# dalek-cryptography/curve25519-dalek

Hardware: NVIDIA H100
Metric: Pippenger MSM points/sec (higher is better)
Workload: dtype exact integers: f64 limbs (radix 2^51, FP64 pipe) in the bucket kernel, u32 limbs (radix 2^25.5) elsewhere

## Files before the change

### curve25519_dalek_b200/csrc/fe64.cuh

```cuda
#pragma once
#include <stdint.h>

#include "fe.cuh"

struct fe64 { double v[5]; };

#define FE64_E52 0x4330000000000000LL
#define FE64_TWO52 4503599627370496.0
#define FE64_TWO51 2251799813685248.0

#if defined(__CUDA_ARCH__)
#define FE64_DEV 1
#else
#define FE64_DEV 0
#include <assert.h>
#include <math.h>
#include <string.h>
#endif

FE_HD void fe64_0(fe64 &h) { for (int i = 0; i < 5; i++) h.v[i] = 0.0; }
FE_HD void fe64_1(fe64 &h) { h.v[0] = 1.0; for (int i = 1; i < 5; i++) h.v[i] = 0.0; }

FE_HD void fe64_add(fe64 &h, const fe64 &f, const fe64 &g)
{
// ... 207 lines not shown
    }
}

FE_HD void fe64_to_fe(fe &o, const fe64 &f)
{
    uint64_t l[5];
#pragma unroll
    for (int k = 0; k < 5; k++) {
        long long r = (long long)f.v[k];
        l[k] = (uint64_t)(r + (k == 0 ? (1LL << 54) - 152 : (1LL << 54) - 8));
    }
    uint64_t c[10];
#pragma unroll
    for (int i = 0; i < 5; i++) { c[2 * i] = l[i] & FE_M26; c[2 * i + 1] = l[i] >> 26; }
    fe_carry64(o, c);
}

FE_HD void fe64_from_fe(fe64 &h, const fe &f)
{
    uint32_t w[8];
    fe_tobytes_words(w, f);
    fe64 t; fe64_frombytes_words(t, w);
    fe64_carry(h, t);
}

FE_HD void fe64_pow22501(fe64 &t19, fe64 &t3, const fe64 &z)
{
    fe64 t0, t1, t2, t5, t6, t7, t9, t13, t15;
    fe64_sq(t0, z);
    fe64_sqn(t1, t0, 2);
// ... 33 lines not shown
```

### curve25519_dalek_b200/csrc/msm.cu

```cuda
#include <algorithm>
#include <cstdio>
#include <utility>
#include <vector>

#include "../../include/dalek_b200.h"
#include "engine.h"
#include "ge64.cuh"
#include "warp4.cuh"
#include "warp4_f64.cuh"

static inline unsigned cdiv(size_t a, unsigned b) { return (unsigned)((a + b - 1) / b); }

int ws_reserve(dalek_b200_ctx *ctx, DevBuf &b, size_t bytes)
{
    if (bytes <= b.cap) return 0;
    if (b.p) { cudaFree(b.p); b.p = nullptr; b.cap = 0; }
    size_t want = bytes + bytes / 8 + 256;
    cudaError_t e = cudaMalloc(&b.p, want);
    if (e != cudaSuccess) {
        ctx->last_error = std::string("cudaMalloc: ") + cudaGetErrorString(e);
        (void)cudaGetLastError();
        return DALEK_E_NOMEM;
    }
    b.cap = want;
// ... 46 lines not shown
    ge_niels nl; ge_affine_to_niels(nl, P.X, P.Y);
    ge_niels_packed pk; ge_niels_pack(pk, nl);
    out[i] = pk;
}

#define PREP_THREADS 256
#define PREP_PER_THREAD 4
#define PREP_GROUP (PREP_THREADS * PREP_PER_THREAD)
#define PREP_NW (PREP_THREADS / 32)

__device__ __forceinline__ void load_coord_f64(fe64 &h, const uint64_t *__restrict__ src)
{
    uint64_t l[5];
#pragma unroll
    for (int k = 0; k < 5; k++) l[k] = __ldg(src + k);
    fe t; fe_from_limbs51(t, l);
    fe64_from_fe_limbs(h, t);
}
__device__ __forceinline__ void store_coord(uint4 *o, const fe64 &v, uint32_t ok, uint32_t c)
{
    fe f;
    uint32_t w[8];
    fe64_to_fe(f, v); fe_tobytes_words(w, f);
#pragma unroll
    for (int q = 0; q < 8; q++) w[q] = ok ? w[q] : (q == 0 ? c : 0u);
    o[0] = make_uint4(w[0], w[1], w[2], w[3]);
    o[1] = make_uint4(w[4], w[5], w[6], w[7]);
}
__device__ __forceinline__ uint32_t load_z(fe64 &h, const uint64_t *__restrict__ in, size_t i)
{
    uint64_t l[5];
#pragma unroll
    for (int k = 0; k < 5; k++) l[k] = __ldg(in + 20 * i + 10 + k);
    fe t; fe_from_limbs51(t, l);
    fe64_from_fe_limbs(h, t);
    return 1u - (uint32_t)fe_iszero(t);
}
__device__ __forceinline__ void fe64_shfl_up(fe64 &o, const fe64 &f, int d)
{
#pragma unroll
    for (int k = 0; k < 5; k++) o.v[k] = __shfl_up_sync(0xffffffffu, f.v[k], d);
}
__device__ __forceinline__ void fe64_shfl_down(fe64 &o, const fe64 &f, int d)
{
#pragma unroll
    for (int k = 0; k < 5; k++) o.v[k] = __shfl_down_sync(0xffffffffu, f.v[k], d);
}
__device__ __forceinline__ void fe64_shfl_xor(fe64 &o, const fe64 &f, int m)
{
#pragma unroll
    for (int k = 0; k < 5; k++) o.v[k] = __shfl_xor_sync(0xffffffffu, f.v[k], m);
// ... 43 lines not shown
        if (INVERT) {
            const w20_role r = w20_roles();
            const double inv = w20_invert(w20_limb(all, r.i), r);
#pragma unroll
            for (uint32_t k = 0; k < 5; k++) t.v[k] = w20_shfl(inv, k);
        } else {
            t = *tot_inv;
        }
        fe64_mul(t, t, b); fe64_mul(t, t, a);
        if (lane < nw) s_warp[lane] = t;
    }
    __syncthreads();
    fe64_mul(inv, s_warp[warp], below); fe64_mul(inv, inv, above);
}

__global__ void __launch_bounds__(PREP_THREADS, 2)
k_prep_zprod(const uint64_t *__restrict__ in, fe64 *__restrict__ prod, size_t n)
{
    __shared__ fe64 s_warp[PREP_NW];
    const uint32_t tid = threadIdx.x, lane = tid & 31, warp = tid >> 5;
    const size_t g0 = (size_t)blockIdx.x * PREP_GROUP + tid;
    fe64 z[PREP_PER_THREAD], acc, t;
    uint32_t ok[PREP_PER_THREAD];
#pragma unroll
    for (int k = 0; k < PREP_PER_THREAD; k++) {
        const size_t i = g0 + (size_t)k * PREP_THREADS;
        if (i < n) ok[k] = load_z(z[k], in, i); else { ok[k] = 0; fe64_1(z[k]); }
    }
    acc = z[0];
    if (!ok[0]) fe64_1(acc);
#pragma unroll
    for (int k = 1; k < PREP_PER_THREAD; k++) { fe64_mul(t, acc, z[k]); fe64_cmov(acc, t, ok[k]); }
    warp_product(t, acc, 32);
    if (lane == 0) s_warp[warp] = t;
    __syncthreads();
    if (warp == 0) {
        if (lane < PREP_NW) acc = s_warp[lane]; else fe64_1(acc);
        warp_product(t, acc, PREP_NW);
        if (lane == 0) prod[blockIdx.x] = t;
    }
}

__global__ void __launch_bounds__(PREP_THREADS)
k_prep_invert(fe64 *__restrict__ prod, fe64 *__restrict__ pre, uint32_t G)
{
    __shared__ fe64 s_warp[PREP_NW];
    const uint32_t per = (G + blockDim.x - 1) / blockDim.x, b = min(threadIdx.x * per, G), e = min(b + per, G);
    fe64 acc, inv, t;
    fe64_1(acc);
    for (uint32_t k = b; k < e; k++) { fe64_mul(acc, acc, prod[k]); pre[k] = acc; }
    block_inverse<true>(inv, acc, s_warp, nullptr);
    for (uint32_t k = e; k-- > b;) {
        const fe64 x = prod[k];
        if (k > b) fe64_mul(t, inv, pre[k - 1]); else t = inv;
        prod[k] = t;
        fe64_mul(inv, inv, x);
    }
}

__global__ void __launch_bounds__(PREP_THREADS, 2)
k_prep_finish(const uint64_t *__restrict__ in, const fe64 *__restrict__ ginv, ge_niels_packed *__restrict__ out, size_t n)
{
    __shared__ fe64 s_warp[PREP_NW];
    __shared__ fe64 s_pre[PREP_PER_THREAD - 1][PREP_THREADS];
    const uint32_t tid = threadIdx.x;
    const size_t g0 = (size_t)blockIdx.x * PREP_GROUP + tid;
    fe64 acc, inv;
    uint32_t nz = 0;
    fe64_1(acc);
#pragma unroll 1
    for (int k = 0; k < PREP_PER_THREAD; k++) {
        const size_t i = g0 + (size_t)k * PREP_THREADS;
// ... 53 lines not shown
int msm_prepare_points_on(dalek_b200_ctx *ctx, cudaStream_t st, const void *d_in, int point_fmt, size_t n, void *d_out, int *d_bad,
                          int kind)
{
    if (n == 0) return 0;
    if (point_fmt == DALEK_POINTS_COMPRESSED) {
        if (ctx->opt_decompress_f64) k_prep_compressed<1><<<cdiv(n, 128), 128, 0, st>>>((const uint4 *)d_in, (ge_niels_packed *)d_out, n, d_bad);
        else k_prep_compressed<0><<<cdiv(n, 128), 128, 0, st>>>((const uint4 *)d_in, (ge_niels_packed *)d_out, n, d_bad);
    } else if (point_fmt == DALEK_POINTS_RISTRETTO) {
        if (ctx->opt_decompress_f64) k_prep_ristretto<1><<<cdiv(n, 128), 128, 0, st>>>((const uint32_t *)d_in, (ge_niels_packed *)d_out, n, d_bad);
        else k_prep_ristretto<0><<<cdiv(n, 128), 128, 0, st>>>((const uint32_t *)d_in, (ge_niels_packed *)d_out, n, d_bad);
    } else if (kind == PK_PNIELS) {
        k_prep_extended_pniels<<<cdiv(n, 128), 128, 0, st>>>((const uint64_t *)d_in, (ge_pniels_packed *)d_out, n);
    } else {
        const unsigned G = cdiv(n, PREP_GROUP);
        int rc;
        if ((rc = ws_reserve(ctx, ctx->ws[WS_PREP_PROD], 2 * (size_t)G * sizeof(fe64)))) return rc;
        fe64 *prod = (fe64 *)ctx->ws[WS_PREP_PROD].p;
        k_prep_zprod<<<G, PREP_THREADS, 0, st>>>((const uint64_t *)d_in, prod, n);
        k_prep_invert<<<1, PREP_THREADS, 0, st>>>(prod, prod + G, G);
        k_prep_finish<<<G, PREP_THREADS, 0, st>>>((const uint64_t *)d_in, prod, (ge_niels_packed *)d_out, n);
        ctx->launches += 2;
    }
    ctx->launches++;
    CUDA_TRY(ctx, cudaGetLastError());
    return 0;
}

int msm_prepare_points(dalek_b200_ctx *ctx, const void *d_in, int point_fmt, size_t n, void *d_out, int *d_bad, int kind)
{
    return msm_prepare_points_on(ctx, ctx->stream, d_in, point_fmt, n, d_out, d_bad, kind);
}

int msm_window_count_for_bits(int c) { return 256 / c + 1; }

int msm_choose_window_bits(const dalek_b200_ctx *ctx, size_t n)
{
// ... 270 lines not shown
            warp_claim(out, r[u].y, k < m);
        }
    }
    __syncthreads();
    for (uint32_t f = threadIdx.x; f < nf; f += SORT_THREADS)
        if (out[f]) out[f] = h[f] + atomicAdd(&fill[b0 + f], out[f]);
    __syncthreads();
    for (uint32_t k0 = 0; k0 < m; k0 += SORT_THREADS) {
        const uint32_t k = k0 + threadIdx.x;
        const uint2 r = k < m ? recs[k] : make_uint2(0, 0);
        const uint32_t pos = warp_claim(out, r.y, k < m);
        if (k < m) dst[pos] = r.x;
    }
}

#define SCAN_PART 4096u
__global__ void __launch_bounds__(1024) k_scan_partial(const uint32_t *__restrict__ in, uint32_t nbuckets, uint32_t parts,
                                                       uint32_t *__restrict__ part_sums)
{
    __shared__ uint32_t sh[32];
    uint32_t w = blockIdx.x / parts, part = blockIdx.x % parts;
    const uint32_t *src = in + (size_t)w * nbuckets;
    uint32_t base = part * SCAN_PART + threadIdx.x * 4, sum = 0;
#pragma unroll
    for (int k = 0; k < 4; k++) if (base + k < nbuckets) sum += src[base + k];
    for (int d = 16; d > 0; d >>= 1) sum += __shfl_down_sync(0xffffffffu, sum, d);
    if ((threadIdx.x & 31) == 0) sh[threadIdx.x >> 5] = sum;
    __syncthreads();
    if (threadIdx.x < 32) {
        uint32_t v = sh[threadIdx.x];
        for (int d = 16; d > 0; d >>= 1) v += __shfl_down_sync(0xffffffffu, v, d);
        if (threadIdx.x == 0) part_sums[blockIdx.x] = v;
    }
}
__global__ void k_scan_bases(uint32_t *__restrict__ part_sums, uint32_t parts)
{
    if (threadIdx.x) return;
    uint32_t *p = part_sums + (size_t)blockIdx.x * parts, run = 0;
    for (uint32_t k = 0; k < parts; k++) { uint32_t v = p[k]; p[k] = run; run += v; }
}
__global__ void __launch_bounds__(1024) k_scan_apply(const uint32_t *__restrict__ in, const uint32_t *__restrict__ part_base,
                                                     uint32_t nbuckets, uint32_t parts, uint32_t *__restrict__ out)
{
    __shared__ uint32_t sh[32];
    uint32_t w = blockIdx.x / parts, part = blockIdx.x % parts;
    const uint32_t *src = in + (size_t)w * nbuckets;
    uint32_t *dst = out + (size_t)w * nbuckets;
    uint32_t base = part * SCAN_PART + threadIdx.x * 4;
    uint32_t v[4], sum = 0;
#pragma unroll
    for (int k = 0; k < 4; k++) { v[k] = base + k < nbuckets ? src[base + k] : 0; sum += v[k]; }
    uint32_t incl = sum;
    for (int d = 1; d < 32; d <<= 1) { uint32_t t = __shfl_up_sync(0xffffffffu, incl, d); if ((threadIdx.x & 31) >= d) incl += t; }
    if ((threadIdx.x & 31) == 31) sh[threadIdx.x >> 5] = incl;
    __syncthreads();
    if (threadIdx.x < 32) {
        uint32_t x = sh[threadIdx.x], inc2 = x;
        for (int d = 1; d < 32; d <<= 1) { uint32_t t = __shfl_up_sync(0xffffffffu, inc2, d); if (threadIdx.x >= d) inc2 += t; }
        sh[threadIdx.x] = inc2 - x;
    }
    __syncthreads();
    uint32_t run = part_base[blockIdx.x] + sh[threadIdx.x >> 5] + incl - sum;
#pragma unroll
    for (int k = 0; k < 4; k++) { if (base + k < nbuckets) dst[base + k] = run; run += v[k]; }
}

#define TASK_LEN_MIN 64u
static uint32_t msm_task_len(size_t n, int nwin, uint32_t nb)
{
    const size_t total_buckets = (size_t)nwin * nb;
    const size_t want = total_buckets >= ((size_t)1 << 18) ? 2 * (n / nb) : (n * (size_t)nwin) >> 18;
    uint32_t len = TASK_LEN_MIN;
    while (len < want && len < (1u << 22)) len <<= 1;
    return len;
}
#ifndef ACC_MIN_BLOCKS
#define ACC_MIN_BLOCKS 4
#endif

__global__ void k_task_count(const uint32_t *__restrict__ counts, uint32_t total_buckets, uint32_t task_len,
                             uint32_t *__restrict__ ntasks, uint32_t *__restrict__ heavy)
{
    uint32_t t = blockIdx.x * blockDim.x + threadIdx.x;
    if (t >= total_buckets) return;
    uint32_t c = counts[t];
    uint32_t k = c <= task_len ? 1u : (c + task_len - 1) / task_len;
    ntasks[t] = k;
    if (k > 1) heavy[1 + atomicAdd(&heavy[0], 1u)] = t;
}

__global__ void k_task_bases(const uint32_t *__restrict__ ntasks, const uint32_t *__restrict__ task_off, uint32_t nbuckets,
                             int nwin, uint32_t *__restrict__ win_base )
{
    if (blockIdx.x || threadIdx.x) return;
    uint32_t run = 0;
    for (int w = 0; w < nwin; w++) {
        win_base[w] = run;
        size_t last = (size_t)w * nbuckets + nbuckets - 1;
        run += task_off[last] + ntasks[last];
    }
    win_base[nwin] = run;
}

__global__ void k_task_fill(const uint32_t *__restrict__ ntasks, const uint32_t *__restrict__ task_off,
                            const uint32_t *__restrict__ win_base, uint32_t nbuckets, uint32_t total_buckets,
                            uint2 *__restrict__ tasks)
{
    uint32_t t = blockIdx.x * blockDim.x + threadIdx.x;
    if (t >= total_buckets) return;
    uint32_t w = t / nbuckets;
    uint32_t base = win_base[w] + task_off[t], k = ntasks[t];
    for (uint32_t j = 0; j < k; j++) tasks[base + j] = make_uint2(t, j);
}

#define TASK_BINS 256u
__device__ __forceinline__ uint32_t task_key(uint32_t len, uint32_t task_len)
{
    return (uint32_t)(((uint64_t)len * (TASK_BINS - 1) + task_len - 1) / task_len);
}
__device__ __forceinline__ uint32_t task_length(const uint2 tk, const uint32_t *__restrict__ counts, uint32_t task_len)
{
    return min(task_len, counts[tk.x] - tk.y * task_len);
}

__global__ void __launch_bounds__(256)
k_task_hist(const uint2 *__restrict__ tasks, const uint32_t *__restrict__ counts, const uint32_t *__restrict__ total_ptr,
            uint32_t task_len, uint32_t *__restrict__ hist)
{
    __shared__ uint32_t sh[TASK_BINS];
    sh[threadIdx.x] = 0;
    __syncthreads();
    const uint32_t p = blockIdx.x * blockDim.x + threadIdx.x;
    if (p < *total_ptr) atomicAdd(&sh[task_key(task_length(tasks[p], counts, task_len), task_len)], 1u);
    __syncthreads();
    if (sh[threadIdx.x]) atomicAdd(&hist[threadIdx.x], sh[threadIdx.x]);
}

__global__ void __launch_bounds__(256) k_task_scan(const uint32_t *__restrict__ hist, uint32_t *__restrict__ start)
{
    __shared__ uint32_t sh[TASK_BINS];
    const uint32_t k = TASK_BINS - 1 - threadIdx.x;
    sh[threadIdx.x] = hist[k];
    __syncthreads();
    for (uint32_t d = 1; d < TASK_BINS; d <<= 1) {
        uint32_t v = threadIdx.x >= d ? sh[threadIdx.x - d] : 0;
        __syncthreads();
        sh[threadIdx.x] += v;
        __syncthreads();
    }
    start[k] = sh[threadIdx.x] - hist[k];
}

__global__ void __launch_bounds__(256)
k_task_scatter(const uint2 *__restrict__ tasks, const uint32_t *__restrict__ counts, const uint32_t *__restrict__ total_ptr,
               uint32_t task_len, const uint32_t *__restrict__ start, uint32_t *__restrict__ cursor, uint32_t *__restrict__ order)
{
    __shared__ uint32_t cnt[TASK_BINS], base[TASK_BINS];
    cnt[threadIdx.x] = 0;
    __syncthreads();
    const uint32_t p = blockIdx.x * blockDim.x + threadIdx.x;
    const bool live = p < *total_ptr;
    uint32_t key = 0, rank = 0;
    if (live) { key = task_key(task_length(tasks[p], counts, task_len), task_len); rank = atomicAdd(&cnt[key], 1u); }
    __syncthreads();
    if (cnt[threadIdx.x]) base[threadIdx.x] = start[threadIdx.x] + atomicAdd(&cursor[threadIdx.x], cnt[threadIdx.x]);
    __syncthreads();
    if (live) order[base[key] + rank] = p;
}

__device__ __forceinline__ void load_p3(ge_p3 &p, const ge_p3_raw *src)
{
    const uint4 *s = reinterpret_cast<const uint4 *>(src);
    ge_p3_raw r;
#pragma unroll
    for (int q = 0; q < 10; q++) { uint4 v = s[q]; r.w[4 * q] = v.x; r.w[4 * q + 1] = v.y; r.w[4 * q + 2] = v.z; r.w[4 * q + 3] = v.w; }
    ge_p3_load_raw(p, r);
}

template <int F64, int TMA>
__global__ void __launch_bounds__(128, ACC_MIN_BLOCKS)
k_bucket_accumulate(const ge_niels_packed *__restrict__ points, const uint32_t *__restrict__ sorted,
                    const uint32_t *__restrict__ counts, const uint32_t *__restrict__ offsets,
                    const uint32_t *__restrict__ ntasks, const uint2 *__restrict__ tasks, const uint32_t *__restrict__ order,
                    const uint32_t *__restrict__ win_base, int w0, int w1, size_t n, uint32_t nbuckets, uint32_t task_len,
                    ge_p3_raw *__restrict__ buckets, ge_p3_raw *__restrict__ task_sums, int first)
{
    constexpr int NQ = sizeof(ge_niels_packed) / 16;
    constexpr int TSTRIDE = NQ * 16 + 16;
    __shared__ uint4 s_pts[(F64 && !TMA) ? 2 : 1][(F64 && !TMA) ? NQ : 1][(F64 && !TMA) ? 128 : 1];
    __shared__ __align__(16) unsigned char s_bulk[(F64 && TMA) ? 2 : 1][(F64 && TMA) ? 128 : 1][(F64 && TMA) ? TSTRIDE : 16];
    __shared__ __align__(8) unsigned long long s_bar[(F64 && TMA) ? 2 : 1][(F64 && TMA) ? 128 : 1];
    const uint32_t total_tasks = win_base[w1];
    const uint32_t slot = blockIdx.x * 128u + threadIdx.x;
    if (slot >= total_tasks) return;
    const uint32_t p = order[slot];
    const uint2 tk = tasks[p];
    const uint32_t t = tk.x, w = t / nbuckets;
    const uint32_t cnt = counts[t], start = tk.y * task_len;
    const uint32_t len = min(task_len, cnt - start);
    const bool split = ntasks[t] != 1;
    if (!first && len == 0) return;
    const bool fold_old = !first && !split;
    const uint32_t *idx = sorted + (size_t)w * n + offsets[t] + start;
    ge_p3 acc;
    if (F64) {
        ge64_p3 acc64;
        if (fold_old) {
// ... 69 lines not shown
#pragma unroll
        for (int q = 0; q < 6; q++) { uint4 v = __ldg(src + q); pk.w[4 * q] = v.x; pk.w[4 * q + 1] = v.y; pk.w[4 * q + 2] = v.z; pk.w[4 * q + 3] = v.w; }
        ge_niels nl; ge_niels_unpack(nl, pk);
        ge_madd(acc, acc, nl, neg);
    }
    }
    ge_p3_raw r; ge_p3_store_raw(r, acc);
    uint4 *o = reinterpret_cast<uint4 *>(!split ? buckets + t : task_sums + p);
#pragma unroll
    for (int q = 0; q < 10; q++) o[q] = make_uint4(r.w[4 * q], r.w[4 * q + 1], r.w[4 * q + 2], r.w[4 * q + 3]);
}


__global__ void __launch_bounds__(128)
k_heavy_fixup(const uint32_t *__restrict__ heavy, const uint32_t *__restrict__ ntasks, const uint32_t *__restrict__ task_off,
              const uint32_t *__restrict__ win_base, uint32_t nbuckets, uint32_t w0, uint32_t w1,
              const ge_p3_raw *__restrict__ task_sums, ge_p3_raw *__restrict__ buckets, int first)
{
    const uint32_t lane = threadIdx.x & 31, role = lane & 3, grp = lane >> 2;
    const uint32_t nwarps = (gridDim.x * blockDim.x) >> 5;
    const uint32_t nheavy = heavy[0];
    for (uint32_t h = (blockIdx.x * blockDim.x + threadIdx.x) >> 5; h < nheavy; h += nwarps) {
        uint32_t tb = heavy[1 + h];
        if (tb / nbuckets < w0 || tb / nbuckets >= w1) continue;
        uint32_t kk = ntasks[tb];
        uint32_t base = win_base[tb / nbuckets] + task_off[tb];
        w4_point acc, x;
        if (first || grp != 0) w4_identity(acc); else w4_load(acc, buckets + tb);
        for (uint32_t j0 = 0; j0 < kk; j0 += 8) {
            uint32_t j = j0 + grp;
            if (j < kk) w4_load(x, task_sums + base + j); else w4_identity(x);
            w4_add(acc, x, role);
        }
        for (int d = 16; d >= 4; d >>= 1) { w4_shfl_down(x, acc, d); w4_add(acc, x, role); }
        if (grp == 0) w4_store(buckets + tb, acc, role);
    }
}

__device__ __forceinline__ void load_p3_f64(ge64_p3 &o, const ge_p3_raw *src)
{
    ge_p3 q; load_p3(q, src);
// ... 137 lines not shown
        lg++;
    return c - 1 - lg;
}

int msm_accumulate_chunk(dalek_b200_ctx *ctx, const uint32_t *d_scalars, const ge_niels_packed *d_points, size_t n,
                         int c, bool first, int active_windows, size_t flat, cudaEvent_t points_ready)
{
    const int nwin_d = msm_window_count_for_bits(c);
    const int nact = active_windows > 0 && active_windows < nwin_d ? active_windows : nwin_d;
    const int nwin = flat ? 1 : nwin_d;
    const uint32_t nb = 1u << (c - 1);
    const size_t total_buckets = (size_t)nwin * nb;
    const uint32_t task_len = flat ? msm_task_len(n * (size_t)nact, 1, nb) : msm_task_len(n, nact, nb);
    const size_t max_tasks = total_buckets + (std::max<size_t>(1, n) * nact) / task_len + 1;
    const size_t max_heavy = (std::max<size_t>(1, n) * nact) / task_len + 1;
    const uint32_t parts = (nb + SCAN_PART - 1) / SCAN_PART;
    const int F = msm_sort_fine_bits(flat ? n * (size_t)nact : n, c, flat ? 1 : nact);
    const uint32_t nc = nb >> F;
    cudaStream_t st = ctx->stream;
    int rc;
    if ((rc = ws_reserve(ctx, ctx->ws[WS_MSM_COUNTS], (total_buckets + (size_t)nwin * nc + 1 + max_heavy) * 4))) return rc;
    if ((rc = ws_reserve(ctx, ctx->ws[WS_MSM_OFFSETS], (total_buckets + (size_t)nwin * parts + 2 * (size_t)nwin * nc + nwin) * 4))) return rc;
    if ((rc = ws_reserve(ctx, ctx->ws[WS_MSM_NTASKS], total_buckets * 4))) return rc;
    if ((rc = ws_reserve(ctx, ctx->ws[WS_MSM_TASK_OFF], total_buckets * 4 + (nwin + 1) * 4))) return rc;
    if ((rc = ws_reserve(ctx, ctx->ws[WS_MSM_TASKS], max_tasks * 8))) return rc;
    if ((rc = ws_reserve(ctx, ctx->ws[WS_MSM_TASK_SUMS], max_tasks * sizeof(ge_p3_raw)))) return rc;
    if ((rc = ws_reserve(ctx, ctx->ws[WS_MSM_TASK_ORDER], (3 * TASK_BINS + max_tasks) * 4))) return rc;
    if ((rc = ws_reserve(ctx, ctx->ws[WS_MSM_DIGITS], std::max<size_t>(1, n) * nact * 8))) return rc;
    if ((rc = ws_reserve(ctx, ctx->ws[WS_MSM_SORTED], std::max<size_t>(1, n) * nact * 4))) return rc;
    if ((rc = ws_reserve(ctx, ctx->ws[WS_MSM_BUCKETS], total_buckets * sizeof(ge_p3_raw)))) return rc;
    uint32_t *counts = (uint32_t *)ctx->ws[WS_MSM_COUNTS].p, *offsets = (uint32_t *)ctx->ws[WS_MSM_OFFSETS].p;
    uint32_t *ntasks = (uint32_t *)ctx->ws[WS_MSM_NTASKS].p, *task_off = (uint32_t *)ctx->ws[WS_MSM_TASK_OFF].p;
    uint32_t *win_base = task_off + total_buckets;
    uint32_t *ccount = counts + total_buckets, *heavy = ccount + (size_t)nwin * nc;
    uint32_t *part_sums = offsets + total_buckets, *ccursor = part_sums + (size_t)nwin * parts;
    uint32_t *xpre = ccursor + (size_t)nwin * nc, *xtot = xpre + (size_t)nwin * nc;
    uint2 *tasks = (uint2 *)ctx->ws[WS_MSM_TASKS].p;
    uint32_t *t_hist = (uint32_t *)ctx->ws[WS_MSM_TASK_ORDER].p, *t_cursor = t_hist + TASK_BINS, *t_start = t_cursor + TASK_BINS;
    uint32_t *order = t_start + TASK_BINS;
    ge_p3_raw *task_sums = (ge_p3_raw *)ctx->ws[WS_MSM_TASK_SUMS].p;
    uint2 *records = (uint2 *)ctx->ws[WS_MSM_DIGITS].p;
    uint32_t *sorted = (uint32_t *)ctx->ws[WS_MSM_SORTED].p;
    ge_p3_raw *buckets = (ge_p3_raw *)ctx->ws[WS_MSM_BUCKETS].p;

    const size_t part_smem = SORT_TILE * 8 + (2 * (size_t)nc + 33) * 4;
    const size_t fine_smem = SORT_FINE_CAP * 12 + ((1u << F) + 33) * 4;
    if (part_smem > SORT_PART_SMEM_MAX || fine_smem > SORT_FINE_SMEM_MAX) {
        ctx->last_error = "msm_accumulate_chunk: digit sort needs more shared memory than its bound";
        return DALEK_E_CUDA;
    }
    if (!ctx->sort_attr_set) {
        CUDA_TRY(ctx, cudaFuncSetAttribute(k_sort_partition, cudaFuncAttributeMaxDynamicSharedMemorySize, (int)SORT_PART_SMEM_MAX));
        CUDA_TRY(ctx, cudaFuncSetAttribute(k_sort_fine, cudaFuncAttributeMaxDynamicSharedMemorySize, (int)SORT_FINE_SMEM_MAX));
        ctx->sort_attr_set = true;
    }
    CUDA_TRY(ctx, cudaMemsetAsync(ccount, 0, ((size_t)nwin * nc + 1) * 4, st));
    CUDA_TRY(ctx, cudaMemsetAsync(t_hist, 0, 2 * TASK_BINS * 4, st));
    if (n) {
        k_sort_count<<<cdiv(n, SORT_COUNT_TILE), SORT_THREADS, 0, st>>>((const uint4 *)d_scalars, n, c, nact, F, nc, flat ? 1 : 0, ccount);
        ctx->launches++;
    }
    k_sort_bins_scan<<<nwin, SORT_THREADS, 0, st>>>(ccount, nc, F, nb, ccursor, xpre, xtot, counts, ntasks);
    if (n) {
        k_sort_partition<<<cdiv(n, SORT_TILE), SORT_THREADS, part_smem, st>>>((const uint4 *)d_scalars, n, c, nact, F, nc, nb, flat,
                                                                              ccount, ccursor, records, counts);
        ctx->launches++;
        CUDA_TRY(ctx, cudaGetLastError());
    }
    const size_t extra = n * (size_t)nact / SORT_FINE_CAP;
    k_sort_fine<<<(unsigned)(nwin * nc + extra), SORT_THREADS, fine_smem, st>>>(records, ccount, ccursor, xpre, xtot, n, F, nc, nb,
                                                                               (uint32_t)nwin, flat ? 1 : 0, counts, offsets, sorted, ntasks);
    CUDA_TRY(ctx, cudaGetLastError());
    k_task_count<<<cdiv(total_buckets, 256), 256, 0, st>>>(counts, (uint32_t)total_buckets, task_len, ntasks, heavy);
    k_scan_partial<<<nwin * parts, 1024, 0, st>>>(ntasks, nb, parts, part_sums);
    k_scan_bases<<<nwin, 32, 0, st>>>(part_sums, parts);
    k_scan_apply<<<nwin * parts, 1024, 0, st>>>(ntasks, part_sums, nb, parts, task_off);
    k_task_bases<<<1, 32, 0, st>>>(ntasks, task_off, nb, nwin, win_base);
    k_task_fill<<<cdiv(total_buckets, 256), 256, 0, st>>>(ntasks, task_off, win_base, nb, (uint32_t)total_buckets, tasks);
    k_task_hist<<<cdiv(max_tasks, 256), 256, 0, st>>>(tasks, counts, win_base + nwin, task_len, t_hist);
    k_task_scan<<<1, 256, 0, st>>>(t_hist, t_start);
    k_task_scatter<<<cdiv(max_tasks, 256), 256, 0, st>>>(tasks, counts, win_base + nwin, task_len, t_start, t_cursor, order);
    ctx->launches += 11;
    if (points_ready) CUDA_TRY(ctx, cudaStreamWaitEvent(st, points_ready, 0));
    if (first) CUDA_TRY(ctx, cudaEventRecord(ctx->ev_a, st));
    {
        const unsigned grid = cdiv(max_tasks, 128);
        const int f = first ? 1 : 0;
#define LAUNCH_ACC(F64_, TMA_) k_bucket_accumulate<F64_, TMA_><<<grid, 128, 0, st>>>(d_points, sorted, counts, offsets, ntasks, tasks, order, win_base, 0, nwin, n, nb, task_len, buckets, task_sums, f)
        const bool tma = ctx->opt_field_f64 && ctx->opt_acc_tma;
        if (tma) LAUNCH_ACC(1, 1); else if (ctx->opt_field_f64) LAUNCH_ACC(1, 0); else LAUNCH_ACC(0, 0);
#undef LAUNCH_ACC
        k_heavy_fixup<<<ctx->sm_count * 4, 128, 0, st>>>(heavy, ntasks, task_off, win_base, nb, 0u, (uint32_t)nwin, task_sums, buckets, f);
        ctx->launches += 2;
    }
    CUDA_TRY(ctx, cudaEventRecord(ctx->ev_b, st));
    ctx->last_kernel_launches = first ? 1 : ctx->last_kernel_launches + 1;
    CUDA_TRY(ctx, cudaGetLastError());
    return 0;
}

int msm_reduce_finish(dalek_b200_ctx *ctx, int c, ge_p3_raw *d_windows, MsmResult *d_result, bool flat)
{
    const int nwin = flat ? 1 : msm_window_count_for_bits(c);
    const int desc_key = c + (flat ? 64 : 0);
    const uint32_t nb = 1u << (c - 1);
    cudaStream_t st = ctx->stream;
    int rc;
// ... 76 lines not shown
```

Baseline: 373.4 million.

## Fuse task-list construction into decoupled-lookback kernel and merge prep inversion into zprod

Replaces the nine small task-scheduling kernels (count, three-stage scan, bases, fill, hist, scan, scatter) with two kernels. One builds per-bucket task counts, a global exclusive scan using decoupled lookback, the task list and the histogram in a single pass. The other fuses the histogram scan with the scatter into the processing order. The prep path folds the single-block group inversion into the last block of k_prep_zprod using an atomic ticket, and adds direct radix-2^51 load and tobytes helpers that skip the u32 field round-trip. The aim is to cut launch count and short serial kernels, at the cost of spin-wait lookback and a serialized final block.

Measured after the change: 374.3 million (median of 6 runs). About the same (+0.2%).

```diff
diff --git a/curve25519_dalek_b200/csrc/fe64.cuh b/curve25519_dalek_b200/csrc/fe64.cuh
--- a/curve25519_dalek_b200/csrc/fe64.cuh
+++ b/curve25519_dalek_b200/csrc/fe64.cuh
@@ -245,6 +245,43 @@
 #pragma unroll
     for (int i = 0; i < 5; i++) { c[2 * i] = l[i] & FE_M26; c[2 * i + 1] = l[i] >> 26; }
     fe_carry64(o, c);
+}
+
+FE_HD void fe64_tobytes_words(uint32_t w[8], const fe64 &f)
+{
+    const uint64_t M51 = (1ull << 51) - 1;
+    uint64_t l[5];
+#pragma unroll
+    for (int k = 0; k < 5; k++) l[k] = (uint64_t)((long long)f.v[k] + (k == 0 ? (1LL << 54) - 152 : (1LL << 54) - 8));
+#pragma unroll
+    for (int k = 0; k < 4; k++) { l[k + 1] += l[k] >> 51; l[k] &= M51; }
+    l[0] += 19 * (l[4] >> 51); l[4] &= M51;
+    uint64_t q = (l[0] + 19) >> 51;
+#pragma unroll
+    for (int k = 1; k < 5; k++) q = (l[k] + q) >> 51;
+    l[0] += 19 * q;
+#pragma unroll
+    for (int k = 0; k < 4; k++) { l[k + 1] += l[k] >> 51; l[k] &= M51; }
+    l[4] &= M51;
+    const uint64_t o[4] = {l[0] | (l[1] << 51), (l[1] >> 13) | (l[2] << 38), (l[2] >> 26) | (l[3] << 25), (l[3] >> 39) | (l[4] << 12)};
+#pragma unroll
+    for (int k = 0; k < 4; k++) { w[2 * k] = (uint32_t)o[k]; w[2 * k + 1] = (uint32_t)(o[k] >> 32); }
+}
+
+FE_HD void fe64_from_limbs51(fe64 &h, const uint64_t l[5])
+{
+    const uint64_t M51 = (1ull << 51) - 1;
+    fe64 t;
+#pragma unroll
+    for (int k = 0; k < 5; k++) {
+        const uint64_t v = (l[k] & M51) + (k == 0 ? 19 * (l[4] >> 51) : l[k - 1] >> 51);
+#if FE64_DEV
+        t.v[k] = __longlong_as_double((long long)v | FE64_E52) - FE64_TWO52;
+#else
+        t.v[k] = (double)v;
+#endif
+    }
+    fe64_carry(h, t);
 }
 
 FE_HD void fe64_from_fe(fe64 &h, const fe &f)
diff --git a/curve25519_dalek_b200/csrc/msm.cu b/curve25519_dalek_b200/csrc/msm.cu
--- a/curve25519_dalek_b200/csrc/msm.cu
+++ b/curve25519_dalek_b200/csrc/msm.cu
@@ -84,14 +84,12 @@
     uint64_t l[5];
 #pragma unroll
     for (int k = 0; k < 5; k++) l[k] = __ldg(src + k);
-    fe t; fe_from_limbs51(t, l);
-    fe64_from_fe_limbs(h, t);
+    fe64_from_limbs51(h, l);
 }
 __device__ __forceinline__ void store_coord(uint4 *o, const fe64 &v, uint32_t ok, uint32_t c)
 {
-    fe f;
     uint32_t w[8];
-    fe64_to_fe(f, v); fe_tobytes_words(w, f);
+    fe64_tobytes_words(w, v);
 #pragma unroll
     for (int q = 0; q < 8; q++) w[q] = ok ? w[q] : (q == 0 ? c : 0u);
     o[0] = make_uint4(w[0], w[1], w[2], w[3]);
@@ -99,12 +97,12 @@
 }
 __device__ __forceinline__ uint32_t load_z(fe64 &h, const uint64_t *__restrict__ in, size_t i)
 {
-    uint64_t l[5];
-#pragma unroll
-    for (int k = 0; k < 5; k++) l[k] = __ldg(in + 20 * i + 10 + k);
-    fe t; fe_from_limbs51(t, l);
-    fe64_from_fe_limbs(h, t);
-    return 1u - (uint32_t)fe_iszero(t);
+    load_coord_f64(h, in + 20 * i + 10);
+    uint32_t w[8], d = 0;
+    fe64_tobytes_words(w, h);
+#pragma unroll
+    for (int q = 0; q < 8; q++) d |= w[q];
+    return d != 0;
 }
 __device__ __forceinline__ void fe64_shfl_up(fe64 &o, const fe64 &f, int d)
 {
@@ -178,10 +176,27 @@
     fe64_mul(inv, s_warp[warp], below); fe64_mul(inv, inv, above);
 }
 
+__device__ __forceinline__ void prep_invert_groups(fe64 *__restrict__ prod, fe64 *__restrict__ pre, uint32_t G, fe64 *s_warp)
+{
+    const uint32_t per = (G + blockDim.x - 1) / blockDim.x, b = min(threadIdx.x * per, G), e = min(b + per, G);
+    auto load = [&](uint32_t k) { fe64 x; for (int q = 0; q < 5; q++) x.v[q] = __ldcg(&prod[k].v[q]); return x; };
+    fe64 acc, inv, t;
+    fe64_1(acc);
+    for (uint32_t k = b; k < e; k++) { fe64_mul(acc, acc, load(k)); pre[k] = acc; }
+    block_inverse<true>(inv, acc, s_warp, nullptr);
+    for (uint32_t k = e; k-- > b;) {
+        const fe64 x = load(k);
+        if (k > b) fe64_mul(t, inv, pre[k - 1]); else t = inv;
+        prod[k] = t;
+        fe64_mul(inv, inv, x);
+    }
+}
+
 __global__ void __launch_bounds__(PREP_THREADS, 2)
-k_prep_zprod(const uint64_t *__restrict__ in, fe64 *__restrict__ prod, size_t n)
+k_prep_zprod(const uint64_t *__restrict__ in, fe64 *__restrict__ prod, fe64 *__restrict__ pre, uint32_t *__restrict__ done, size_t n)
 {
     __shared__ fe64 s_warp[PREP_NW];
+    __shared__ uint32_t s_last;
     const uint32_t tid = threadIdx.x, lane = tid & 31, warp = tid >> 5;
     const size_t g0 = (size_t)blockIdx.x * PREP_GROUP + tid;
     fe64 z[PREP_PER_THREAD], acc, t;
@@ -201,25 +216,16 @@
     if (warp == 0) {
         if (lane < PREP_NW) acc = s_warp[lane]; else fe64_1(acc);
         warp_product(t, acc, PREP_NW);
-        if (lane == 0) prod[blockIdx.x] = t;
-    }
-}
-
-__global__ void __launch_bounds__(PREP_THREADS)
-k_prep_invert(fe64 *__restrict__ prod, fe64 *__restrict__ pre, uint32_t G)
-{
-    __shared__ fe64 s_warp[PREP_NW];
-    const uint32_t per = (G + blockDim.x - 1) / blockDim.x, b = min(threadIdx.x * per, G), e = min(b + per, G);
-    fe64 acc, inv, t;
-    fe64_1(acc);
-    for (uint32_t k = b; k < e; k++) { fe64_mul(acc, acc, prod[k]); pre[k] = acc; }
-    block_inverse<true>(inv, acc, s_warp, nullptr);
-    for (uint32_t k = e; k-- > b;) {
-        const fe64 x = prod[k];
-        if (k > b) fe64_mul(t, inv, pre[k - 1]); else t = inv;
-        prod[k] = t;
-        fe64_mul(inv, inv, x);
-    }
+        if (lane == 0) {
+            prod[blockIdx.x] = t;
+            __threadfence();
+            s_last = atomicAdd(done, 1u) == gridDim.x - 1;
+        }
+    }
+    __syncthreads();
+    if (!s_last) return;
+    __threadfence();
+    prep_invert_groups(prod, pre, gridDim.x, s_warp);
 }
 
 __global__ void __launch_bounds__(PREP_THREADS, 2)
@@ -303,12 +309,13 @@
     } else {
         const unsigned G = cdiv(n, PREP_GROUP);
         int rc;
-        if ((rc = ws_reserve(ctx, ctx->ws[WS_PREP_PROD], 2 * (size_t)G * sizeof(fe64)))) return rc;
+        if ((rc = ws_reserve(ctx, ctx->ws[WS_PREP_PROD], 2 * (size_t)G * sizeof(fe64) + 4))) return rc;
         fe64 *prod = (fe64 *)ctx->ws[WS_PREP_PROD].p;
-        k_prep_zprod<<<G, PREP_THREADS, 0, st>>>((const uint64_t *)d_in, prod, n);
-        k_prep_invert<<<1, PREP_THREADS, 0, st>>>(prod, prod + G, G);
+        uint32_t *done = (uint32_t *)(prod + 2 * (size_t)G);
+        CUDA_TRY(ctx, cudaMemsetAsync(done, 0, 4, st));
+        k_prep_zprod<<<G, PREP_THREADS, 0, st>>>((const uint64_t *)d_in, prod, prod + G, done, n);
         k_prep_finish<<<G, PREP_THREADS, 0, st>>>((const uint64_t *)d_in, prod, (ge_niels_packed *)d_out, n);
-        ctx->launches += 2;
+        ctx->launches++;
     }
     ctx->launches++;
     CUDA_TRY(ctx, cudaGetLastError());
@@ -609,57 +616,6 @@
     }
 }
 
-#define SCAN_PART 4096u
-__global__ void __launch_bounds__(1024) k_scan_partial(const uint32_t *__restrict__ in, uint32_t nbuckets, uint32_t parts,
-                                                       uint32_t *__restrict__ part_sums)
-{
-    __shared__ uint32_t sh[32];
-    uint32_t w = blockIdx.x / parts, part = blockIdx.x % parts;
-    const uint32_t *src = in + (size_t)w * nbuckets;
-    uint32_t base = part * SCAN_PART + threadIdx.x * 4, sum = 0;
-#pragma unroll
-    for (int k = 0; k < 4; k++) if (base + k < nbuckets) sum += src[base + k];
-    for (int d = 16; d > 0; d >>= 1) sum += __shfl_down_sync(0xffffffffu, sum, d);
-    if ((threadIdx.x & 31) == 0) sh[threadIdx.x >> 5] = sum;
-    __syncthreads();
-    if (threadIdx.x < 32) {
-        uint32_t v = sh[threadIdx.x];
-        for (int d = 16; d > 0; d >>= 1) v += __shfl_down_sync(0xffffffffu, v, d);
-        if (threadIdx.x == 0) part_sums[blockIdx.x] = v;
-    }
-}
-__global__ void k_scan_bases(uint32_t *__restrict__ part_sums, uint32_t parts)
-{
-    if (threadIdx.x) return;
-    uint32_t *p = part_sums + (size_t)blockIdx.x * parts, run = 0;
-    for (uint32_t k = 0; k < parts; k++) { uint32_t v = p[k]; p[k] = run; run += v; }
-}
-__global__ void __launch_bounds__(1024) k_scan_apply(const uint32_t *__restrict__ in, const uint32_t *__restrict__ part_base,
-                                                     uint32_t nbuckets, uint32_t parts, uint32_t *__restrict__ out)
-{
-    __shared__ uint32_t sh[32];
-    uint32_t w = blockIdx.x / parts, part = blockIdx.x % parts;
-    const uint32_t *src = in + (size_t)w * nbuckets;
-    uint32_t *dst = out + (size_t)w * nbuckets;
-    uint32_t base = part * SCAN_PART + threadIdx.x * 4;
-    uint32_t v[4], sum = 0;
-#pragma unroll
-    for (int k = 0; k < 4; k++) { v[k] = base + k < nbuckets ? src[base + k] : 0; sum += v[k]; }
-    uint32_t incl = sum;
-    for (int d = 1; d < 32; d <<= 1) { uint32_t t = __shfl_up_sync(0xffffffffu, incl, d); if ((threadIdx.x & 31) >= d) incl += t; }
-    if ((threadIdx.x & 31) == 31) sh[threadIdx.x >> 5] = incl;
-    __syncthreads();
-    if (threadIdx.x < 32) {
-        uint32_t x = sh[threadIdx.x], inc2 = x;
-        for (int d = 1; d < 32; d <<= 1) { uint32_t t = __shfl_up_sync(0xffffffffu, inc2, d); if (threadIdx.x >= d) inc2 += t; }
-        sh[threadIdx.x] = inc2 - x;
-    }
-    __syncthreads();
-    uint32_t run = part_base[blockIdx.x] + sh[threadIdx.x >> 5] + incl - sum;
-#pragma unroll
-    for (int k = 0; k < 4; k++) { if (base + k < nbuckets) dst[base + k] = run; run += v[k]; }
-}
-
 #define TASK_LEN_MIN 64u
 static uint32_t msm_task_len(size_t n, int nwin, uint32_t nb)
 {
@@ -673,41 +629,6 @@
 #define ACC_MIN_BLOCKS 4
 #endif
 
-__global__ void k_task_count(const uint32_t *__restrict__ counts, uint32_t total_buckets, uint32_t task_len,
-                             uint32_t *__restrict__ ntasks, uint32_t *__restrict__ heavy)
-{
-    uint32_t t = blockIdx.x * blockDim.x + threadIdx.x;
-    if (t >= total_buckets) return;
-    uint32_t c = counts[t];
-    uint32_t k = c <= task_len ? 1u : (c + task_len - 1) / task_len;
-    ntasks[t] = k;
-    if (k > 1) heavy[1 + atomicAdd(&heavy[0], 1u)] = t;
-}
-
-__global__ void k_task_bases(const uint32_t *__restrict__ ntasks, const uint32_t *__restrict__ task_off, uint32_t nbuckets,
-                             int nwin, uint32_t *__restrict__ win_base )
-{
-    if (blockIdx.x || threadIdx.x) return;
-    uint32_t run = 0;
-    for (int w = 0; w < nwin; w++) {
-        win_base[w] = run;
-        size_t last = (size_t)w * nbuckets + nbuckets - 1;
-        run += task_off[last] + ntasks[last];
-    }
-    win_base[nwin] = run;
-}
-
-__global__ void k_task_fill(const uint32_t *__restrict__ ntasks, const uint32_t *__restrict__ task_off,
-                            const uint32_t *__restrict__ win_base, uint32_t nbuckets, uint32_t total_buckets,
-                            uint2 *__restrict__ tasks)
-{
-    uint32_t t = blockIdx.x * blockDim.x + threadIdx.x;
-    if (t >= total_buckets) return;
-    uint32_t w = t / nbuckets;
-    uint32_t base = win_base[w] + task_off[t], k = ntasks[t];
-    for (uint32_t j = 0; j < k; j++) tasks[base + j] = make_uint2(t, j);
-}
-
 #define TASK_BINS 256u
 __device__ __forceinline__ uint32_t task_key(uint32_t len, uint32_t task_len)
 {
@@ -718,49 +639,98 @@
     return min(task_len, counts[tk.x] - tk.y * task_len);
 }
 
-__global__ void __launch_bounds__(256)
-k_task_hist(const uint2 *__restrict__ tasks, const uint32_t *__restrict__ counts, const uint32_t *__restrict__ total_ptr,
-            uint32_t task_len, uint32_t *__restrict__ hist)
-{
-    __shared__ uint32_t sh[TASK_BINS];
-    sh[threadIdx.x] = 0;
-    __syncthreads();
-    const uint32_t p = blockIdx.x * blockDim.x + threadIdx.x;
-    if (p < *total_ptr) atomicAdd(&sh[task_key(task_length(tasks[p], counts, task_len), task_len)], 1u);
-    __syncthreads();
-    if (sh[threadIdx.x]) atomicAdd(&hist[threadIdx.x], sh[threadIdx.x]);
-}
-
-__global__ void __launch_bounds__(256) k_task_scan(const uint32_t *__restrict__ hist, uint32_t *__restrict__ start)
-{
-    __shared__ uint32_t sh[TASK_BINS];
-    const uint32_t k = TASK_BINS - 1 - threadIdx.x;
-    sh[threadIdx.x] = hist[k];
-    __syncthreads();
-    for (uint32_t d = 1; d < TASK_BINS; d <<= 1) {
-        uint32_t v = threadIdx.x >= d ? sh[threadIdx.x - d] : 0;
+#define TASK_TILE 4096u
+#define TASK_THREADS 512u
+#define TASK_ORDER_PER 4u
+#define TILE_AGGREGATE (1ull << 32)
+#define TILE_PREFIX (2ull << 32)
+
+__global__ void __launch_bounds__(TASK_THREADS)
+k_task_lists(const uint32_t *__restrict__ counts, uint32_t total_buckets, uint32_t task_len, uint32_t *__restrict__ ntasks,
+             uint32_t *__restrict__ heavy, uint32_t *__restrict__ task_off, uint2 *__restrict__ tasks,
+             uint32_t *__restrict__ hist, uint32_t *__restrict__ ticket, unsigned long long *__restrict__ status,
+             uint32_t *__restrict__ total)
+{
+    __shared__ uint32_t v[TASK_TILE], h[TASK_BINS], scr[33];
+    __shared__ uint32_t s_tile, s_base;
+    if (threadIdx.x == 0) s_tile = atomicAdd(ticket, 1u);
+    for (uint32_t k = threadIdx.x; k < TASK_BINS; k += TASK_THREADS) h[k] = 0;
+    __syncthreads();
+    const uint32_t tile = s_tile, b0 = tile * TASK_TILE, len = min(TASK_TILE, total_buckets - b0);
+    for (uint32_t k = threadIdx.x; k < len; k += TASK_THREADS) {
+        const uint32_t t = b0 + k, cnt = counts[t];
+        const uint32_t m = cnt <= task_len ? 1u : (cnt + task_len - 1) / task_len;
+        v[k] = m;
+        ntasks[t] = m;
+        if (m > 1) { heavy[1 + atomicAdd(&heavy[0], 1u)] = t; atomicAdd(&h[TASK_BINS - 1], m - 1); }
+        atomicAdd(&h[task_key(cnt - (m - 1) * task_len, task_len)], 1u);
+    }
+    const uint32_t sum = block_excl_scan(v, len, scr);
+    if (threadIdx.x < 32) {
+        const uint32_t lane = threadIdx.x;
+        uint32_t pre = 0;
+        if (tile > 0 && lane == 0) atomicExch(status + tile, TILE_AGGREGATE | sum);
+        for (int j0 = (int)tile - 1; j0 >= 0; j0 -= 32) {
+            const int j = j0 - (int)lane;
+            unsigned long long x = TILE_PREFIX;
+            if (j >= 0) do { x = atomicAdd(status + j, 0ull); } while (x < TILE_AGGREGATE);
+            const uint32_t pmask = __ballot_sync(0xffffffffu, x >= TILE_PREFIX);
+            const uint32_t stop = pmask ? __ffs(pmask) - 1 : 31;
+            uint32_t v = lane <= stop ? (uint32_t)x : 0u;
+            for (int d = 16; d > 0; d >>= 1) v += __shfl_xor_sync(0xffffffffu, v, d);
+            pre += v;
+            if (pmask) break;
+        }
+        if (lane == 0) {
+            atomicExch(status + tile, TILE_PREFIX | (pre + sum));
+            s_base = pre;
+            if (b0 + len == total_buckets) *total = pre + sum;
+        }
+    }
+    __syncthreads();
+    for (uint32_t k = threadIdx.x; k < len; k += TASK_THREADS) {
+        const uint32_t t = b0 + k, base = s_base + v[k], m = (k + 1 < len ? v[k + 1] : sum) - v[k];
+        for (uint32_t j = 0; j < m; j++) tasks[base + j] = make_uint2(t, j);
+        if (m > 1) task_off[t] = base;
+    }
+    for (uint32_t k = threadIdx.x; k < TASK_BINS; k += TASK_THREADS)
+        if (h[k]) atomicAdd(&hist[k], h[k]);
+}
+
+__global__ void __launch_bounds__(TASK_BINS)
+k_task_order(const uint2 *__restrict__ tasks, const uint32_t *__restrict__ counts, const uint32_t *__restrict__ total_ptr,
+             uint32_t task_len, const uint32_t *__restrict__ hist, uint32_t *__restrict__ cursor, uint32_t *__restrict__ order)
+{
+    __shared__ uint32_t sh[TASK_BINS], start[TASK_BINS], cnt[TASK_BINS];
+    {
+        const uint32_t k = TASK_BINS - 1 - threadIdx.x;
+        const uint32_t x = hist[k];
+        sh[threadIdx.x] = x;
+        cnt[threadIdx.x] = 0;
         __syncthreads();
-        sh[threadIdx.x] += v;
-        __syncthreads();
-    }
-    start[k] = sh[threadIdx.x] - hist[k];
-}
-
-__global__ void __launch_bounds__(256)
-k_task_scatter(const uint2 *__restrict__ tasks, const uint32_t *__restrict__ counts, const uint32_t *__restrict__ total_ptr,
-               uint32_t task_len, const uint32_t *__restrict__ start, uint32_t *__restrict__ cursor, uint32_t *__restrict__ order)
-{
-    __shared__ uint32_t cnt[TASK_BINS], base[TASK_BINS];
-    cnt[threadIdx.x] = 0;
-    __syncthreads();
-    const uint32_t p = blockIdx.x * blockDim.x + threadIdx.x;
-    const bool live = p < *total_ptr;
-    uint32_t key = 0, rank = 0;
-    if (live) { key = task_key(task_length(tasks[p], counts, task_len), task_len); rank = atomicAdd(&cnt[key], 1u); }
-    __syncthreads();
-    if (cnt[threadIdx.x]) base[threadIdx.x] = start[threadIdx.x] + atomicAdd(&cursor[threadIdx.x], cnt[threadIdx.x]);
-    __syncthreads();
-    if (live) order[base[key] + rank] = p;
+        for (uint32_t d = 1; d < TASK_BINS; d <<= 1) {
+            const uint32_t y = threadIdx.x >= d ? sh[threadIdx.x - d] : 0;
+            __syncthreads();
+            sh[threadIdx.x] += y;
+            __syncthreads();
+        }
+        start[k] = sh[threadIdx.x] - x;
+    }
+    const uint32_t total = *total_ptr;
+    uint32_t key[TASK_ORDER_PER], rank[TASK_ORDER_PER];
+#pragma unroll
+    for (uint32_t u = 0; u < TASK_ORDER_PER; u++) {
+        const uint32_t p = (blockIdx.x * TASK_ORDER_PER + u) * TASK_BINS + threadIdx.x;
+        if (p < total) { key[u] = task_key(task_length(tasks[p], counts, task_len), task_len); rank[u] = atomicAdd(&cnt[key[u]], 1u); }
+    }
+    __syncthreads();
+    if (cnt[threadIdx.x]) start[threadIdx.x] += atomicAdd(&cursor[threadIdx.x], cnt[threadIdx.x]);
+    __syncthreads();
+#pragma unroll
+    for (uint32_t u = 0; u < TASK_ORDER_PER; u++) {
+        const uint32_t p = (blockIdx.x * TASK_ORDER_PER + u) * TASK_BINS + threadIdx.x;
+        if (p < total) order[start[key[u]] + rank[u]] = p;
+    }
 }
 
 __device__ __forceinline__ void load_p3(ge_p3 &p, const ge_p3_raw *src)
@@ -777,7 +747,7 @@
 k_bucket_accumulate(const ge_niels_packed *__restrict__ points, const uint32_t *__restrict__ sorted,
                     const uint32_t *__restrict__ counts, const uint32_t *__restrict__ offsets,
                     const uint32_t *__restrict__ ntasks, const uint2 *__restrict__ tasks, const uint32_t *__restrict__ order,
-                    const uint32_t *__restrict__ win_base, int w0, int w1, size_t n, uint32_t nbuckets, uint32_t task_len,
+                    const uint32_t *__restrict__ ntotal, size_t n, uint32_t nbuckets, uint32_t task_len,
                     ge_p3_raw *__restrict__ buckets, ge_p3_raw *__restrict__ task_sums, int first)
 {
     constexpr int NQ = sizeof(ge_niels_packed) / 16;
@@ -785,7 +755,7 @@
     __shared__ uint4 s_pts[(F64 && !TMA) ? 2 : 1][(F64 && !TMA) ? NQ : 1][(F64 && !TMA) ? 128 : 1];
     __shared__ __align__(16) unsigned char s_bulk[(F64 && TMA) ? 2 : 1][(F64 && TMA) ? 128 : 1][(F64 && TMA) ? TSTRIDE : 16];
     __shared__ __align__(8) unsigned long long s_bar[(F64 && TMA) ? 2 : 1][(F64 && TMA) ? 128 : 1];
-    const uint32_t total_tasks = win_base[w1];
+    const uint32_t total_tasks = *ntotal;
     const uint32_t slot = blockIdx.x * 128u + threadIdx.x;
     if (slot >= total_tasks) return;
     const uint32_t p = order[slot];
@@ -885,17 +855,13 @@
 
 __global__ void __launch_bounds__(128)
 k_heavy_fixup(const uint32_t *__restrict__ heavy, const uint32_t *__restrict__ ntasks, const uint32_t *__restrict__ task_off,
-              const uint32_t *__restrict__ win_base, uint32_t nbuckets, uint32_t w0, uint32_t w1,
               const ge_p3_raw *__restrict__ task_sums, ge_p3_raw *__restrict__ buckets, int first)
 {
     const uint32_t lane = threadIdx.x & 31, role = lane & 3, grp = lane >> 2;
     const uint32_t nwarps = (gridDim.x * blockDim.x) >> 5;
     const uint32_t nheavy = heavy[0];
     for (uint32_t h = (blockIdx.x * blockDim.x + threadIdx.x) >> 5; h < nheavy; h += nwarps) {
-        uint32_t tb = heavy[1 + h];
-        if (tb / nbuckets < w0 || tb / nbuckets >= w1) continue;
-        uint32_t kk = ntasks[tb];
-        uint32_t base = win_base[tb / nbuckets] + task_off[tb];
+        const uint32_t tb = heavy[1 + h], kk = ntasks[tb], base = task_off[tb];
         w4_point acc, x;
         if (first || grp != 0) w4_identity(acc); else w4_load(acc, buckets + tb);
         for (uint32_t j0 = 0; j0 < kk; j0 += 8) {
@@ -1063,30 +1029,32 @@
     const uint32_t task_len = flat ? msm_task_len(n * (size_t)nact, 1, nb) : msm_task_len(n, nact, nb);
     const size_t max_tasks = total_buckets + (std::max<size_t>(1, n) * nact) / task_len + 1;
     const size_t max_heavy = (std::max<size_t>(1, n) * nact) / task_len + 1;
-    const uint32_t parts = (nb + SCAN_PART - 1) / SCAN_PART;
+    const uint32_t ntiles = cdiv(total_buckets, TASK_TILE);
     const int F = msm_sort_fine_bits(flat ? n * (size_t)nact : n, c, flat ? 1 : nact);
     const uint32_t nc = nb >> F;
     cudaStream_t st = ctx->stream;
     int rc;
     if ((rc = ws_reserve(ctx, ctx->ws[WS_MSM_COUNTS], (total_buckets + (size_t)nwin * nc + 1 + max_heavy) * 4))) return rc;
-    if ((rc = ws_reserve(ctx, ctx->ws[WS_MSM_OFFSETS], (total_buckets + (size_t)nwin * parts + 2 * (size_t)nwin * nc + nwin) * 4))) return rc;
+    if ((rc = ws_reserve(ctx, ctx->ws[WS_MSM_OFFSETS], (total_buckets + 2 * (size_t)nwin * nc + nwin) * 4))) return rc;
     if ((rc = ws_reserve(ctx, ctx->ws[WS_MSM_NTASKS], total_buckets * 4))) return rc;
-    if ((rc = ws_reserve(ctx, ctx->ws[WS_MSM_TASK_OFF], total_buckets * 4 + (nwin + 1) * 4))) return rc;
+    if ((rc = ws_reserve(ctx, ctx->ws[WS_MSM_TASK_OFF], total_buckets * 4))) return rc;
     if ((rc = ws_reserve(ctx, ctx->ws[WS_MSM_TASKS], max_tasks * 8))) return rc;
     if ((rc = ws_reserve(ctx, ctx->ws[WS_MSM_TASK_SUMS], max_tasks * sizeof(ge_p3_raw)))) return rc;
-    if ((rc = ws_reserve(ctx, ctx->ws[WS_MSM_TASK_ORDER], (3 * TASK_BINS + max_tasks) * 4))) return rc;
+    const size_t order_head = (2 * TASK_BINS + 2) * 4 + (size_t)ntiles * 8;
+    if ((rc = ws_reserve(ctx, ctx->ws[WS_MSM_TASK_ORDER], order_head + max_tasks * 4))) return rc;
     if ((rc = ws_reserve(ctx, ctx->ws[WS_MSM_DIGITS], std::max<size_t>(1, n) * nact * 8))) return rc;
     if ((rc = ws_reserve(ctx, ctx->ws[WS_MSM_SORTED], std::max<size_t>(1, n) * nact * 4))) return rc;
     if ((rc = ws_reserve(ctx, ctx->ws[WS_MSM_BUCKETS], total_buckets * sizeof(ge_p3_raw)))) return rc;
     uint32_t *counts = (uint32_t *)ctx->ws[WS_MSM_COUNTS].p, *offsets = (uint32_t *)ctx->ws[WS_MSM_OFFSETS].p;
     uint32_t *ntasks = (uint32_t *)ctx->ws[WS_MSM_NTASKS].p, *task_off = (uint32_t *)ctx->ws[WS_MSM_TASK_OFF].p;
-    uint32_t *win_base = task_off + total_buckets;
     uint32_t *ccount = counts + total_buckets, *heavy = ccount + (size_t)nwin * nc;
-    uint32_t *part_sums = offsets + total_buckets, *ccursor = part_sums + (size_t)nwin * parts;
+    uint32_t *ccursor = offsets + total_buckets;
     uint32_t *xpre = ccursor + (size_t)nwin * nc, *xtot = xpre + (size_t)nwin * nc;
     uint2 *tasks = (uint2 *)ctx->ws[WS_MSM_TASKS].p;
-    uint32_t *t_hist = (uint32_t *)ctx->ws[WS_MSM_TASK_ORDER].p, *t_cursor = t_hist + TASK_BINS, *t_start = t_cursor + TASK_BINS;
-    uint32_t *order = t_start + TASK_BINS;
+    uint32_t *t_hist = (uint32_t *)ctx->ws[WS_MSM_TASK_ORDER].p, *t_cursor = t_hist + TASK_BINS, *t_ticket = t_cursor + TASK_BINS;
+    uint32_t *t_total = t_ticket + 1;
+    unsigned long long *t_status = (unsigned long long *)(t_ticket + 2);
+    uint32_t *order = (uint32_t *)((char *)ctx->ws[WS_MSM_TASK_ORDER].p + order_head);
     ge_p3_raw *task_sums = (ge_p3_raw *)ctx->ws[WS_MSM_TASK_SUMS].p;
     uint2 *records = (uint2 *)ctx->ws[WS_MSM_DIGITS].p;
     uint32_t *sorted = (uint32_t *)ctx->ws[WS_MSM_SORTED].p;
@@ -1104,7 +1072,7 @@
         ctx->sort_attr_set = true;
     }
     CUDA_TRY(ctx, cudaMemsetAsync(ccount, 0, ((size_t)nwin * nc + 1) * 4, st));
-    CUDA_TRY(ctx, cudaMemsetAsync(t_hist, 0, 2 * TASK_BINS * 4, st));
+    CUDA_TRY(ctx, cudaMemsetAsync(t_hist, 0, order_head, st));
     if (n) {
         k_sort_count<<<cdiv(n, SORT_COUNT_TILE), SORT_THREADS, 0, st>>>((const uint4 *)d_scalars, n, c, nact, F, nc, flat ? 1 : 0, ccount);
         ctx->launches++;
@@ -1120,26 +1088,20 @@
     k_sort_fine<<<(unsigned)(nwin * nc + extra), SORT_THREADS, fine_smem, st>>>(records, ccount, ccursor, xpre, xtot, n, F, nc, nb,
                                                                                (uint32_t)nwin, flat ? 1 : 0, counts, offsets, sorted, ntasks);
     CUDA_TRY(ctx, cudaGetLastError());
-    k_task_count<<<cdiv(total_buckets, 256), 256, 0, st>>>(counts, (uint32_t)total_buckets, task_len, ntasks, heavy);
-    k_scan_partial<<<nwin * parts, 1024, 0, st>>>(ntasks, nb, parts, part_sums);
-    k_scan_bases<<<nwin, 32, 0, st>>>(part_sums, parts);
-    k_scan_apply<<<nwin * parts, 1024, 0, st>>>(ntasks, part_sums, nb, parts, task_off);
-    k_task_bases<<<1, 32, 0, st>>>(ntasks, task_off, nb, nwin, win_base);
-    k_task_fill<<<cdiv(total_buckets, 256), 256, 0, st>>>(ntasks, task_off, win_base, nb, (uint32_t)total_buckets, tasks);
-    k_task_hist<<<cdiv(max_tasks, 256), 256, 0, st>>>(tasks, counts, win_base + nwin, task_len, t_hist);
-    k_task_scan<<<1, 256, 0, st>>>(t_hist, t_start);
-    k_task_scatter<<<cdiv(max_tasks, 256), 256, 0, st>>>(tasks, counts, win_base + nwin, task_len, t_start, t_cursor, order);
-    ctx->launches += 11;
+    k_task_lists<<<ntiles, TASK_THREADS, 0, st>>>(counts, (uint32_t)total_buckets, task_len, ntasks, heavy, task_off, tasks, t_hist,
+                                                  t_ticket, t_status, t_total);
+    k_task_order<<<cdiv(max_tasks, TASK_ORDER_PER * TASK_BINS), TASK_BINS, 0, st>>>(tasks, counts, t_total, task_len, t_hist, t_cursor, order);
+    ctx->launches += 4;
     if (points_ready) CUDA_TRY(ctx, cudaStreamWaitEvent(st, points_ready, 0));
     if (first) CUDA_TRY(ctx, cudaEventRecord(ctx->ev_a, st));
     {
         const unsigned grid = cdiv(max_tasks, 128);
         const int f = first ? 1 : 0;
-#define LAUNCH_ACC(F64_, TMA_) k_bucket_accumulate<F64_, TMA_><<<grid, 128, 0, st>>>(d_points, sorted, counts, offsets, ntasks, tasks, order, win_base, 0, nwin, n, nb, task_len, buckets, task_sums, f)
+#define LAUNCH_ACC(F64_, TMA_) k_bucket_accumulate<F64_, TMA_><<<grid, 128, 0, st>>>(d_points, sorted, counts, offsets, ntasks, tasks, order, t_total, n, nb, task_len, buckets, task_sums, f)
         const bool tma = ctx->opt_field_f64 && ctx->opt_acc_tma;
         if (tma) LAUNCH_ACC(1, 1); else if (ctx->opt_field_f64) LAUNCH_ACC(1, 0); else LAUNCH_ACC(0, 0);
 #undef LAUNCH_ACC
-        k_heavy_fixup<<<ctx->sm_count * 4, 128, 0, st>>>(heavy, ntasks, task_off, win_base, nb, 0u, (uint32_t)nwin, task_sums, buckets, f);
+        k_heavy_fixup<<<ctx->sm_count * 4, 128, 0, st>>>(heavy, ntasks, task_off, task_sums, buckets, f);
         ctx->launches += 2;
     }
     CUDA_TRY(ctx, cudaEventRecord(ctx->ev_b, st));
```
